# chenjianqu/dynamic_vins

Hardware: AMD Instinct MI355X
Metric: stereo frames/sec (track+BA) (higher is better)
Workload: dtype f64; 1 GPU; synthetic 1280x720 stereo @20 Hz + IMU @200 Hz, ZED intrinsics with distortion, figure-8 in a textured box room, max_cnt 250, min_dist 25, flow_back 1, 10 solver iterations, BA + marginalization on every frame; mode=raw, config=zed, parallelism=replicas x1 (independent sequences, no collective), landmarks_in_window=266, features_per_frame=250, warmup_requested=5, gpu_max_hw_queues=4, frames=resident in HBM before the timed region

## Files before the change

dynamic_vins_amd/csrc/be_api.hip:

```cpp
#include <algorithm>
#include "be_host.h"

static_assert(sizeof(dv_ba_factor) == sizeof(BeFactor), "public/private factor layouts must match");
static_assert(sizeof(dv_ba_lm) == sizeof(BeLm), "public/private landmark layouts must match");
static_assert(sizeof(dv_ba_prior) == sizeof(BePriorHdr), "public/private prior layouts must match");

int be_ensure(dv_ctx* ctx, int nfac) {
    BeWork& w = ctx->be;
    if (w.ready && nfac <= w.fac_cap) return 0;
    const int fac_cap = std::max(nfac, BE_MAX_LM * BE_MAX_OBS_FACTORS);
    size_t off = 0;
    auto take = [&](size_t bytes) { size_t o = off; off += (bytes + 255) / 256 * 256; return o; };
    const size_t n = BE_MAX_STATE;
    size_t o_ctl = take(sizeof(BeCtl)), o_x = take(sizeof(BeState)), o_imu = take(sizeof(BeImu) * BE_WIN), o_pr = take(sizeof(BePriorHdr)), o_i = take(4 * 4 * n),
           o_mt = take(4 * BE_MARG_TAB_INTS), o_lm = take(sizeof(BeLm) * BE_MAX_LM), o_fac = take(sizeof(BeFactor) * (size_t)fac_cap);
    const size_t upload_bytes = off;
    size_t o_c = take(sizeof(BeState)),
           o_pA = take(8 * (size_t)BE_MAX_PRIOR * BE_MAX_PRIOR), o_pb = take(8 * BE_MAX_PRIOR),
           o_pA2 = take(8 * (size_t)BE_MAX_PRIOR * BE_MAX_PRIOR), o_pb2 = take(8 * BE_MAX_PRIOR), o_ms = take(64), o_c0 = take(64),
           o_pk = take(8 * (size_t)BE_PK_SIZE * BE_PK_STRIDE), o_io = take(8 * (size_t)BE_WIN * IMU_OUT_STRIDE), o_po = take(8 * (BE_MAX_PRIOR + 1)),
           o_cc = take(8 * (BE_MAX_LM + BE_WIN + 1)), o_ob = take(4 * BE_MAX_LM), o_hd = take(8 * n * n), o_sc = take(8 * n * n), o_g = take(8 * 2 * n),
           o_pk1 = take(8 * (size_t)BE_PK_SIZE * BE_PK_STRIDE), o_io1 = take(8 * (size_t)BE_WIN * IMU_OUT_STRIDE), o_po1 = take(8 * (BE_MAX_PRIOR + 1)),
           o_hd1 = take(8 * n * n), o_sc1 = take(8 * n * n), o_g1 = take(8 * 2 * n),
           o_v = take(8 * 4 * n), o_vl = take(8 * 4 * (size_t)BE_MAX_LM);
// ... 267 lines not shown
    BeEvalArgs ea{};
    ea.ctl = w.ctl; ea.x = w.x; ea.cand = w.cand; ea.fac = w.fac; ea.lm = w.lm; ea.imu = w.imu; ea.prior = w.prior; ea.priorA = w.priorA; ea.priorb = w.priorb;
    ea.dims = d; ea.g_norm = P->g_norm; ea.cand_cost = w.cand_cost; ea.lm_obs = w.lm_obs; ea.prior_c0 = w.prior_c0 + w.prior_cur;
    ea.lm_lo = 0; ea.lm_hi = P->nlm;
    if (P->free_blocks & 3) {
        if (ctx->dist.transport != 0) DV_FAIL("dv_ba_solve: free extrinsic / td blocks are not built for the landmark-sharded window");
        if (xt.on) {
            DV_CHECK(w.xpk_buf.ensure(2 * 8 * (size_t)BX_SIZE * BE_PK_STRIDE));
            xt.xpk[0] = (double*)w.xpk_buf.p; xt.xpk[1] = xt.xpk[0] + (size_t)BX_SIZE * BE_PK_STRIDE;
        }
    }
    BeShard sh{};
    if (ctx->dist.transport != 0) {
        const DvDist& dd = ctx->dist;
        sh.on = 1; sh.rank = dd.rank; sh.world = dd.world;
        sh.cap = std::max(1, (P->nlm + dd.world - 1) / dd.world);
        sh.lo = std::min(P->nlm, dd.rank * sh.cap); sh.hi = std::min(P->nlm, sh.lo + sh.cap);
        sh.len = BE_XS_LEN;
        sh.xsend = (double*)dd.xsend.p; sh.xrecv = (const double*)dd.xrecv.p;
        sh.qf[0] = (double*)dd.qf.p; sh.qf[1] = sh.qf[0] + BE_QF_LEN;
        ea.lm_lo = sh.lo; ea.lm_hi = sh.hi;
    }
    for (int k = 0; k < 2; ++k) { ea.packets[k] = w.packets[k]; ea.imu_out[k] = w.imu_out[k]; ea.prior_out[k] = w.prior_out[k]; }
    BeSolveArgs sa{};
    sa.ctl = w.ctl; sa.x = w.x; sa.cand = w.cand; sa.lm = w.lm; sa.imu = w.imu; sa.prior = w.prior; sa.priorA = w.priorA; sa.dims = d;
    sa.cand_cost = w.cand_cost; sa.lm_obs = w.lm_obs;
    for (int k = 0; k < 2; ++k) { sa.packets[k] = w.packets[k]; sa.imu_out[k] = w.imu_out[k]; sa.prior_out[k] = w.prior_out[k]; sa.Hd[k] = w.Hd[k]; sa.Sc[k] = w.Sc[k]; sa.gvec[k] = w.gvec[k]; }
    sa.scale_p = w.scale_p; sa.diag_p = w.diag_p; sa.grad_p = w.grad_p; sa.gn_p = w.gn_p; sa.scale_l = w.scale_l; sa.diag_l = w.diag_l; sa.grad_l = w.grad_l; sa.gn_l = w.gn_l;
    sa.prior_col = w.prior_col; sa.col_kind = w.col_kind; sa.col_frame = w.col_frame; sa.col_comp = w.col_comp;
    sa.xnorm2_extra = P->x_norm2_extra; sa.sh = sh; sa.xt = xt;
    sa.ldl_mf16 = 0;
    if (!w.ldl_generic && !(P->free_blocks & 3)) {
        uint8_t plan[64];
        if (be_mf16_plan(d.nstate, plan)) { std::memcpy(sa.ldl_col0, plan, sizeof(plan)); sa.ldl_mf16 = 1; }
    }
    pd.rej_on = false;
    if (fused && fused->want_reject && w.gpu_reject && P->nlm > 0) {
        if (!w.rej_pinned) DV_CHECK(hipHostMalloc((void**)&w.rej_pinned, BE_MAX_LM, hipHostMallocDefault));
        BeRejectArgs& r = pd.rej;
        r.st = w.cand; r.fac = w.fac; r.lm = w.lm; r.nlm = P->nlm; r.nframes = P->nframes; r.focal = fused->rej_focal; r.flags = w.rej_pinned;
        std::memcpy(r.ric, fused->rej_ric, sizeof(r.ric)); std::memcpy(r.tic, fused->rej_tic, sizeof(r.tic));
        r.ex_from_state = (P->free_blocks & 1) ? 1 : 0; r.pad = 0;
        pd.rej_on = true;
    }
    pd.xt = xt; pd.copy_ex_td = (P->free_blocks & 3) != 0;
    pd.ea = ea; pd.sa = sa; pd.fused_present = fused != nullptr; pd.fuse_accept_gauge = fused != nullptr && !ctx->batch && !sh.on ; pd.max_iters = P->max_iters; pd.g_norm = P->g_norm; pd.nframes = P->nframes; pd.use_imu = P->use_imu; pd.nlm = P->nlm;
    pd.want_raw_pose = fused && fused->want_raw_pose;
    if (fused) { std::memcpy(pd.gauge_R0, fused->R0, sizeof(pd.gauge_R0)); std::memcpy(pd.gauge_ypr0, fused->ypr0, sizeof(pd.gauge_ypr0)); std::memcpy(pd.gauge_P0, fused->P0, sizeof(pd.gauge_P0)); }
    pd.do_marg = do_marg; pd.state_bytes = state_bytes; pd.nxt = 1 - w.prior_cur;
    if (eval_only) {
        be_launch_eval(ea, BE_EVAL_X, s); be_launch_eval_ext(ea, xt, BE_EVAL_X, s);
        be_launch_reduce(sa, 0, s); be_launch_reduce_ext(sa, 0, s);
        if (sh.on) { if (be_exchange(ctx, (size_t)sh.len, s)) return -1; be_launch_shard_finalize(sa, 0, s); }
        DV_CHECK(hipGetLastError());
        return 0;
    }
    if (w.debug_hash_log && fused) {
        if (!w.dbg_pinned) DV_CHECK(hipHostMalloc((void**)&w.dbg_pinned, 64, hipHostMallocDefault));
        const size_t up_bytes = w.up_fac + sizeof(BeFactor) * (size_t)P->nfac;
        be_dbg_hash(w.block.p, up_bytes & ~(size_t)7, w.dbg_pinned + 0, s);
        const bool pv = P->prior && P->prior->valid;
        if (pv) { be_dbg_hash(w.priorA, 8 * (size_t)P->prior->n * P->prior->n, w.dbg_pinned + 1, s); be_dbg_hash(w.priorb, 8 * (size_t)P->prior->n, w.dbg_pinned + 2, s); } else { w.dbg_pinned[1] = 0; w.dbg_pinned[2] = 0; }
    }
    const int first_slots = w.debug_short_first_pass ? std::max(1, P->max_iters - 2) : P->max_iters;
    if (ctx->batch && fused && !sh.on) {
        pd.deferred = true; pd.first_slots = first_slots;
        pd.active = true; pd.t_begin = t_begin; pd.t_up = t_up; pd.t_enq = t_up;
// ... 190 lines not shown
```

dynamic_vins_amd/csrc/be_debug.hip:

```cpp
#include <algorithm>
#include "be_host.h"

__global__ __launch_bounds__(256) void be_dbg_hash_kernel(const unsigned long long* __restrict__ p, size_t words, unsigned long long* __restrict__ out) {
    __shared__ unsigned long long sh[256];
    unsigned long long h = 1469598103934665603ull;
    for (size_t i = threadIdx.x; i < words; i += 256) { h ^= p[i]; h *= 1099511628211ull; }
    sh[threadIdx.x] = h;
    __syncthreads();
    if (threadIdx.x == 0) { unsigned long long t = 1469598103934665603ull; for (int k = 0; k < 256; ++k) { t ^= sh[k]; t *= 1099511628211ull; } *out = t; }
}
struct BeDbgJob { const unsigned long long* p[BeWork::DBG_RANGES]; unsigned long long words[BeWork::DBG_RANGES]; unsigned long long* out; };
__global__ __launch_bounds__(256) void be_dbg_hash_multi_kernel(BeDbgJob j) {
    __shared__ unsigned long long sh[256];
    const unsigned long long* p = j.p[blockIdx.x]; const unsigned long long words = j.words[blockIdx.x];
    unsigned long long h = 1469598103934665603ull;
    for (unsigned long long i = threadIdx.x; i < words; i += 256) { h ^= p[i]; h *= 1099511628211ull; }
    sh[threadIdx.x] = h;
    __syncthreads();
    if (threadIdx.x == 0) { unsigned long long t = 1469598103934665603ull; for (int k = 0; k < 256; ++k) { t ^= sh[k]; t *= 1099511628211ull; } j.out[blockIdx.x] = t; }
}
void be_dbg_stage(dv_ctx* c, int it, int kind, hipStream_t s) {
    BeWork& w = c->be;
    if (!w.debug_hash_log || it >= BeWork::DBG_SLOTS) return;
    const bool light = w.debug_hash_light;
// ... 16 lines not shown

extern "C" {

int dv_ba_debug_dev_log(dv_ctx* ctx, unsigned long long* rows7, int cap, int* n_rows) {
    if (!ctx) return -1;
    const int n = (int)(ctx->be.dbg_dev_log.size() / 7);
    if (n_rows) *n_rows = n;
    if (rows7) std::memcpy(rows7, ctx->be.dbg_dev_log.data(), sizeof(unsigned long long) * 7 * (size_t)std::min(n, std::max(cap, 0)));
    return 0;
}

int dv_ba_debug_slot_log(dv_ctx* ctx, unsigned long long* vals, long long cap_vals, long long* n_vals, int* row_len) {
    if (!ctx) return -1;
    const long long n = (long long)ctx->be.dbg_slot_log.size();
    if (n_vals) *n_vals = n;
    if (row_len) *row_len = BeWork::DBG_SLOTS * 5 * BeWork::DBG_RANGES;
    if (vals) std::memcpy(vals, ctx->be.dbg_slot_log.data(), sizeof(unsigned long long) * (size_t)std::min(n, std::max(cap_vals, 0ll)));
    return 0;
}

int dv_debug_set(dv_ctx* ctx, const char* key, int value) {
    if (!ctx || !key) return -1;
    if (std::strcmp(key, "short_first_pass") == 0) { ctx->be.debug_short_first_pass = value != 0; return 0; }
    if (std::strcmp(key, "peer_timeout_ms") == 0) { ctx->dist.peer_timeout_ticks = 100000ll * std::max(value, 1); return 0; }
    if (std::strcmp(key, "batch_single_eval") == 0) { ctx->be.debug_batch_single = (ctx->be.debug_batch_single & ~1) | (value ? 1 : 0); return 0; }
    if (std::strcmp(key, "batch_single_reduce") == 0) { ctx->be.debug_batch_single = (ctx->be.debug_batch_single & ~2) | (value ? 2 : 0); return 0; }
    if (std::strcmp(key, "batch_single_tail") == 0) { ctx->be.debug_batch_single = (ctx->be.debug_batch_single & ~8) | (value ? 8 : 0); return 0; }
    if (std::strcmp(key, "batch_single_solve") == 0) { ctx->be.debug_batch_single = (ctx->be.debug_batch_single & ~4) | (value ? 4 : 0); return 0; }
    if (std::strcmp(key, "hash_light") == 0) { ctx->be.debug_hash_light = value != 0; return 0; }
    if (std::strcmp(key, "hash_log") == 0) { ctx->be.debug_hash_log = value != 0; return 0; }
    if (std::strcmp(key, "wait_tail") == 0) { ctx->be.debug_wait_tail = value != 0; return 0; }
    if (std::strcmp(key, "gpu_reject") == 0) { ctx->be.gpu_reject = value != 0; return 0; }
    if (std::strcmp(key, "ldl_generic") == 0) { ctx->be.ldl_generic = value != 0; return 0; }
    DV_FAIL(std::string("dv_debug_set: unknown key ") + key);
}

}
```

dynamic_vins_amd/csrc/be_mf16.h:

```cpp
#pragma once
#include <hip/hip_runtime.h>
#include <cstdint>
#include "wave_dpp.h"

__device__ __forceinline__ void lds_barrier() { asm volatile("s_waitcnt lgkmcnt(0)\n\ts_barrier" ::: "memory"); }

__device__ __forceinline__ double fast_rcp(double d) {
    double r = __builtin_amdgcn_rcp(d);
    r = __builtin_fma(__builtin_fma(-d, r, 1.0), r, r);
    r = __builtin_fma(__builtin_fma(-d, r, 1.0), r, r);
    return r;
}

__device__ __forceinline__ void wave_lds_sync() { __builtin_amdgcn_fence(__ATOMIC_ACQ_REL, "wavefront"); __builtin_amdgcn_wave_barrier(); }

#define MF_SLOTS 5
#define MF_MAXNB 11
#define MF_RHO 1e300
typedef double mf_d4 __attribute__((ext_vector_type(4)));
__device__ __forceinline__ mf_d4 mf_mfma(double a, double b, mf_d4 c) { return __builtin_amdgcn_mfma_f64_16x16x4f64(a, b, c, 0, 0, 0); }
__device__ __forceinline__ int mf_tix(int I, int J, int NB) { return J * NB - (J * (J - 1)) / 2 + (I - J); }
template <int LANE> __device__ __forceinline__ double mf_rowbc(double v) { return dpp_f64<0x150 + LANE, 0xf>(v); }
__device__ __forceinline__ double mf_sel4(int rho, double v0, double v1, double v2, double v3) {
    const bool b0 = (rho & 1) != 0, b1 = (rho & 2) != 0;
    const double t0 = b0 ? v1 : v0, t1 = b0 ? v3 : v2;
    return b1 ? t1 : t0;
}
__device__ __forceinline__ int mf_wave() { return __builtin_amdgcn_readfirstlane(threadIdx.x >> 6); }
struct MfLds { double* Tl; double* gat; double* dv; double* iv; double* yv; };

template <int Q, bool RR>
__device__ __forceinline__ void mf_diag_substep(mf_d4& T, mf_d4& Wt, double* gat, double* dv16, double* iv16, int c0, double* yk) {
    constexpr int P = 4 * Q;
    const int lane = threadIdx.x & 63, c = lane & 15, rho = lane >> 4;
    gat[lane] = T[Q];
    wave_lds_sync();
    const double g0 = gat[c], g1 = gat[16 + c], g2 = gat[32 + c], g3 = gat[48 + c];
    const double d0 = gat[P], a10 = gat[16 + P], a11 = gat[16 + P + 1], a20 = gat[32 + P], a21 = gat[32 + P + 1], a22 = gat[32 + P + 2];
    const double a30 = gat[48 + P], a31 = gat[48 + P + 1], a32 = gat[48 + P + 2], a33 = gat[48 + P + 3];
    wave_lds_sync();
    const double i0 = RR ? (d0 > 1e-8 ? fast_rcp(d0) : 0.0) : fast_rcp(d0);
    const double l10 = a10 * i0, l20 = a20 * i0, l30 = a30 * i0;
    const double d1 = __builtin_fma(-l10, a10, a11), i1 = RR ? (d1 > 1e-8 ? fast_rcp(d1) : 0.0) : fast_rcp(d1);
    const double t21 = __builtin_fma(-l20, a10, a21), t31 = __builtin_fma(-l30, a10, a31);
    const double l21 = t21 * i1, l31 = t31 * i1;
    const double d2 = __builtin_fma(-l21, t21, __builtin_fma(-l20, a20, a22)), i2 = RR ? (d2 > 1e-8 ? fast_rcp(d2) : 0.0) : fast_rcp(d2);
    const double t32 = __builtin_fma(-l31, t21, __builtin_fma(-l30, a20, a32));
    const double l32 = t32 * i2;
    const double d3 = __builtin_fma(-l32, t32, __builtin_fma(-l31, t31, __builtin_fma(-l30, a30, a33))), i3 = RR ? (d3 > 1e-8 ? fast_rcp(d3) : 0.0) : fast_rcp(d3);
    const double p0 = g0, p1 = __builtin_fma(-p0, l10, g1);
    const double p2 = __builtin_fma(-p1, l21, __builtin_fma(-p0, l20, g2));
    const double p3 = __builtin_fma(-p2, l32, __builtin_fma(-p1, l31, __builtin_fma(-p0, l30, g3)));
    const double lh0 = c > P ? p0 * i0 : 0.0, lh1 = c > P + 1 ? p1 * i1 : 0.0, lh2 = c > P + 2 ? p2 * i2 : 0.0, lh3 = c > P + 3 ? p3 * i3 : 0.0;
    T = mf_mfma(-mf_sel4(rho, lh0, lh1, lh2, lh3), mf_sel4(rho, p0, p1, p2, p3), T);
    const double w20 = __builtin_fma(l21, l10, -l20), w31 = __builtin_fma(l32, l21, -l31);
    const double w30 = __builtin_fma(-l32, w20, __builtin_fma(l31, l10, -l30));
    const double z0 = -__builtin_fma(lh3, w30, __builtin_fma(lh2, w20, __builtin_fma(-lh1, l10, lh0)));
    const double z1 = -__builtin_fma(lh3, w31, __builtin_fma(-lh2, l21, lh1));
    const double z2 = -__builtin_fma(-lh3, l32, lh2);
    const double wq = Wt[Q];
    Wt = mf_mfma(mf_sel4(rho, z0, z1, z2, -lh3), wq, Wt);
    if (lane == 0) {
        mf_d4 dd = { d0, d1, d2, d3 }, ii = { i0, i1, i2, i3 };
        *reinterpret_cast<mf_d4*>(dv16 + P) = dd; *reinterpret_cast<mf_d4*>(iv16 + P) = ii;
    }
    if (lane == c0) { mf_d4 yy = { lh0, lh1, lh2, lh3 }; *reinterpret_cast<mf_d4*>(yk + P) = yy; }
}
template <bool RR = false>
__device__ __forceinline__ void mf_diag_factor(mf_d4& T, const MfLds& m, int k, int NB, int n, int* s_fail) {
    const int lane = threadIdx.x & 63, c = lane & 15, rho = lane >> 4, wave = mf_wave();
    __builtin_amdgcn_s_setprio(3);
    mf_d4 Wt;
#pragma unroll
    for (int r = 0; r < 4; ++r) Wt[r] = (rho + 4 * r == c) ? 1.0 : 0.0;
    double* gat = m.gat + wave * 64;
    const int nv = n - 16 * k, c0 = (nv >= 0 && nv < 16) ? nv : -1;
    mf_diag_substep<0, RR>(T, Wt, gat, m.dv + 16 * k, m.iv + 16 * k, c0, m.yv + 16 * k);
    if (c0 < 0 || c0 >= 4) mf_diag_substep<1, RR>(T, Wt, gat, m.dv + 16 * k, m.iv + 16 * k, c0, m.yv + 16 * k);
    if (c0 < 0 || c0 >= 8) mf_diag_substep<2, RR>(T, Wt, gat, m.dv + 16 * k, m.iv + 16 * k, c0, m.yv + 16 * k);
    if (c0 < 0 || c0 >= 12) mf_diag_substep<3, RR>(T, Wt, gat, m.dv + 16 * k, m.iv + 16 * k, c0, m.yv + 16 * k);
    *reinterpret_cast<mf_d4*>(m.Tl + (size_t)mf_tix(k, k, NB) * 256 + lane * 4) = Wt;
    {
        double* wt = m.gat + 768;
#pragma unroll
        for (int r = 0; r < 4; ++r) wt[((((c & 3) << 4) + rho + 4 * r) << 2) + (c >> 2)] = Wt[r];
    }
    __builtin_amdgcn_s_setprio(0);
}
__device__ __forceinline__ void mf_diag(mf_d4& T, const MfLds& m, int k, int NB, int n, int* s_fail) { mf_diag_factor<false>(T, m, k, NB, n, s_fail); }
__device__ __forceinline__ void mf_slots(const uint8_t* plan, int wave, int NB, int (&sI)[5], int (&sJ)[5]) {
    sI[0] = sJ[0] = wave < NB ? wave : -1;
    const uint32_t w4 = reinterpret_cast<const uint32_t*>(plan)[wave];
#pragma unroll
    for (int s = 1; s < 5; ++s) { const int b = (int)((w4 >> (8 * (s - 1))) & 0xFFu); sI[s] = b == 0xFF ? -1 : (b >> 4); sJ[s] = b == 0xFF ? -1 : (b & 15); }
}

template <bool RR, class After>
__device__ __forceinline__ void mf16_factor_core(mf_d4 (&U)[MF_SLOTS], const uint8_t* plan, int n, const MfLds& m, int* s_fail, After after_update) {
    const int lane = threadIdx.x & 63, wave = mf_wave(), c = lane & 15, rho = lane >> 4;
    const int NB = (n + 16) >> 4, IB = n >> 4, c0 = n & 15;
    int sI[MF_SLOTS], sJ[MF_SLOTS];
    mf_slots(plan, wave, NB, sI, sJ);
    if (wave == 0) mf_diag_factor<RR>(U[0], m, 0, NB, n, s_fail);
    lds_barrier();
    auto panel = [&](mf_d4& T, int I, int k) -> mf_d4 {
        const mf_d4 wf = *reinterpret_cast<const mf_d4*>(m.gat + 768 + lane * 4);
        double ivr[4];
#pragma unroll
        for (int q = 0; q < 4; ++q) ivr[q] = m.iv[16 * k + rho + 4 * q];
        mf_d4 Y = { 0.0, 0.0, 0.0, 0.0 };
#pragma unroll
        for (int q = 0; q < 4; ++q) Y = mf_mfma(wf[q], T[q], Y);
        const mf_d4 Y0 = Y;
#pragma unroll
// ... 39 lines not shown
```

dynamic_vins_amd/csrc/be_solve.hip:

```cpp
#include <hip/hip_runtime.h>
#include <cfloat>
#include <algorithm>
#include <cstring>
#include <cstdlib>
#include "be_kernels.h"
#include "dev_once.h"
#include "wave_dpp.h"
#include "be_mf16.h"

using namespace be;

#ifdef BE_RED_TS
__device__ long long be_red_ts[64];
#define RTS(k) do { if (threadIdx.x == 0) be_red_ts[k] = wall_clock64(); } while (0)
extern "C" int dv_debug_red_ts(long long* out) { return hipMemcpyFromSymbol(out, HIP_SYMBOL(be_red_ts), sizeof(long long) * 64) == hipSuccess ? 0 : -1; }
#else
#define RTS(k) do {} while (0)
#endif
#define RED_THREADS 448
#define RED_PAIRS (BE_NF * (BE_NF + 1) / 2)
__device__ const unsigned char RED_PAIR_TAB[RED_PAIRS] = {
    150, 152, 51, 132, 98, 166, 170, 112, 147, 85, 68, 65, 32, 168, 49, 167, 118, 153, 66, 129, 96, 130, 165, 144, 33, 148, 67, 48, 102, 162, 161, 0, 97,
    133, 50, 16, 101, 134, 17, 119, 99, 84, 114, 64, 80, 100, 163, 160, 145, 149, 115, 131, 82, 164, 81, 151, 113, 117, 116, 128, 34, 136, 83, 169, 146, 135 };
__device__ __forceinline__ void red_pair(int bx, int& fi, int& fj) { const int t = RED_PAIR_TAB[bx]; fi = t >> 4; fj = t & 15; }
// ... 650 lines not shown
    const int NBR = (n + 3) >> 2, bi = i >> 2, bj = j >> 2;
    const bool in = i < n;
    return Sc[in ? (size_t)(bj * NBR - bj * (bj - 1) / 2 + bi - bj) * 16 + (i & 3) * 4 + (j & 3) : 0];
}
__device__ __forceinline__ double mf_finish(double raw, const double* v_s, const double* v_d, const double* rhs, int n, double mu, int i, int j) {
    const int hi = i > j ? i : j, lo = i > j ? j : i, hc = hi < n ? hi : n - 1, lc = lo < n ? lo : n - 1;
    const double s_hi = v_s[hc], s_lo = v_s[lc], d_hi = v_d[hc];
    const double body = s_hi * s_lo * raw + (i == j ? mu * d_hi * d_hi : 0.0);
    const double row_n = lo == n ? MF_RHO : s_lo * rhs[lc];
    return hi < n ? body : (hi == n ? row_n : (hi == lo ? 1.0 : 0.0));
}
__device__ __forceinline__ void mf_prefetch(const double* __restrict__ Sc, const uint8_t* plan, int n, mf_d4 (&U)[5]) {
    const int lane = threadIdx.x & 63, wave = mf_wave(), c = lane & 15, rho = lane >> 4;
    int sI[5], sJ[5];
    mf_slots(plan, wave, (n + 16) >> 4, sI, sJ);
    const int NBR = (n + 3) >> 2;
#pragma unroll
    for (int s = 0; s < 5; ++s) {
        if (sI[s] > sJ[s]) {
            const int i = min(16 * sI[s] + c, n - 1);
            const int lane_off = ((i >> 2) << 4) + ((i & 3) << 2) + rho;
#pragma unroll
            for (int r = 0; r < 4; ++r) {
                const int bj = 4 * sJ[s] + r;
                const int bjc = bj < NBR ? bj : 0;
                U[s][r] = Sc[(size_t)((bjc * NBR - bjc * (bjc - 1) / 2 - bjc) << 4) + lane_off];
            }
        } else {
#pragma unroll
            for (int r = 0; r < 4; ++r) U[s][r] = sI[s] >= 0 ? mf_raw(Sc, n, 16 * sI[s] + c, 16 * sJ[s] + rho + 4 * r) : 0.0;
        }
    }
}
template <class Side, class Side0>
__device__ __forceinline__ bool ldlt_mf16(mf_d4 (&U)[MF_SLOTS], const uint8_t* plan, int n, double mu, const double* v_s, const double* v_d, const double* rhs, const MfLds& m, int* s_fail, Side side, Side0 side0) {
    const int tid = threadIdx.x, lane = tid & 63, wave = mf_wave(), c = lane & 15, rho = lane >> 4;
    const int NB = (n + 16) >> 4, IB = n >> 4, c0 = n & 15;
    int sI[MF_SLOTS], sJ[MF_SLOTS];
    mf_slots(plan, wave, NB, sI, sJ);
    TS(21);
#pragma unroll
    for (int s = 0; s < MF_SLOTS; ++s) {
        if (sI[s] > sJ[s]) {
            const int i = 16 * sI[s] + c;
            const double si = v_s[min(i, n - 1)];
#pragma unroll
            for (int r = 0; r < 4; ++r) {
                const int j = 16 * sJ[s] + rho + 4 * r;
                const double sj = v_s[j];
                const double body = si * sj * U[s][r];
                U[s][r] = i < n ? body : (i == n ? sj * rhs[j] : 0.0);
            }
        } else {
#pragma unroll
            for (int r = 0; r < 4; ++r) U[s][r] = sI[s] >= 0 ? mf_finish(U[s][r], v_s, v_d, rhs, n, mu, 16 * sI[s] + c, 16 * sJ[s] + rho + 4 * r) : 0.0;
        }
    }
    TS(22);
    for (int i = tid; i < 16 * NB; i += SOL_THREADS) m.yv[i] = 0.0;
    if (tid == 0) *s_fail = 0;
#ifdef BE_SOLVE_TS
    if (tid == 0) { be_dbg_ts[19] = 0; be_dbg_ts[20] = 0; be_dbg_ts[32] = 0; be_dbg_ts[33] = 0; be_dbg_ts[34] = 0; be_dbg_ts[35] = 0; }
#endif
    lds_barrier();
    TS(4);
    const int k_side = -1;
    if (wave == 0) { mf_diag(U[0], m, 0, NB, n, s_fail); if (k_side < 0) side0(); }
    else if (k_side < 0) side(0);
    lds_barrier();
#ifdef BE_SOLVE_TS
    long long t_prev = wall_clock64(), acc_panel = 0, acc_update = 0;
    if (tid == 0) be_dbg_ts[16] = t_prev - be_dbg_ts[4];
#endif
    auto panel = [&](mf_d4& T, int I, int k) -> mf_d4 {
        const mf_d4 wf = *reinterpret_cast<const mf_d4*>(m.gat + 768 + lane * 4);
        double ivr[4];
#pragma unroll
        for (int q = 0; q < 4; ++q) ivr[q] = m.iv[16 * k + rho + 4 * q];
        mf_d4 Y = { 0.0, 0.0, 0.0, 0.0 };
#pragma unroll
        for (int q = 0; q < 4; ++q) Y = mf_mfma(wf[q], T[q], Y);
        const mf_d4 Y0 = Y;
#pragma unroll
        for (int r = 0; r < 4; ++r) Y[r] *= ivr[r];
        T = Y;
        *reinterpret_cast<mf_d4*>(m.Tl + (size_t)mf_tix(I, k, NB) * 256 + lane * 4) = Y;
        if (I == IB && c == c0) {
#pragma unroll
            for (int r = 0; r < 4; ++r) m.yv[16 * k + rho + 4 * r] = Y[r];
        }
        return Y0;
    };
    for (int k = 0; k + 1 < NB; ++k) {
        if (wave == k + 1) {
            __builtin_amdgcn_s_setprio(3);
#ifdef BE_SOLVE_TS
            const long long t_c0 = wall_clock64();
#endif
            const mf_d4 Y0 = panel(U[1], k + 1, k);
#ifdef BE_SOLVE_TS
            __builtin_amdgcn_s_waitcnt(0xc07f); const long long t_c1 = wall_clock64();
#endif
#pragma unroll
            for (int q = 0; q < 4; ++q) U[0] = mf_mfma(U[1][q], -Y0[q], U[0]);
#ifdef BE_SOLVE_TS
            asm volatile("s_nop 15\n\ts_nop 3\n\tv_mov_b64 %0, %0" : "+v"(U[0][0])); const long long t_c2 = wall_clock64();
#endif
            if (k + 2 < NB) lds_barrier();
#ifdef BE_SOLVE_TS
            const long long t_u = wall_clock64();
            if (lane == 0) { be_dbg_ts[32] += t_c0 - t_prev; be_dbg_ts[33] += t_c1 - t_c0; be_dbg_ts[34] += t_c2 - t_c1; be_dbg_ts[35] += t_u - t_c2; }
#endif
            mf_diag(U[0], m, k + 1, NB, n, s_fail);
#ifdef BE_SOLVE_TS
            if (lane == 0) { be_dbg_ts[19] += wall_clock64() - t_u; be_dbg_ts[20] += t_u - t_prev; }
#endif
            lds_barrier();
        } else {
#pragma unroll
            for (int s = 1; s < MF_SLOTS; ++s) if (sJ[s] == k) panel(U[s], sI[s], k);
            if (k + 2 < NB) lds_barrier();
#ifdef BE_SOLVE_TS
            { const long long t = wall_clock64(); acc_panel += t - t_prev; t_prev = t; }
#endif
            double dk[4];
// ... 126 lines not shown
        const double xk = lane_bcast(xs, kt - u - 64 * SEG);
        x0 = __builtin_fma(-(SEG == 0 ? m[u] : cr[u][0]), xk, x0);
        if (SEG >= 1) x1 = __builtin_fma(-(SEG == 1 ? m[u] : cr[u][1]), xk, x1);
        if (SEG >= 2) x2 = __builtin_fma(-m[u], xk, x2);
    }
}
template <int SEG, int R>
__device__ __forceinline__ int bs_segment(const double* Lm, int k, int lane, double& x0, double& x1, double& x2) {
    const int kend = 64 * SEG + R - 1;
    double ca[R][3], cb[R][3];
    bs_ld<SEG, R>(Lm, k, lane, ca);
    for (; k >= kend; k -= 2 * R) {
        if (k - R >= kend) bs_ld<SEG, R>(Lm, k - R, lane, cb);
        __builtin_amdgcn_sched_barrier(0);
        bs_ap<SEG, R>(ca, k, lane, x0, x1, x2);
        __builtin_amdgcn_sched_barrier(0);
        if (k - R >= kend) {
            if (k - 2 * R >= kend) bs_ld<SEG, R>(Lm, k - 2 * R, lane, ca);
            __builtin_amdgcn_sched_barrier(0);
            bs_ap<SEG, R>(cb, k - R, lane, x0, x1, x2);
            __builtin_amdgcn_sched_barrier(0);
        }
    }
    return 64 * SEG - 1;
}
template <int ROWS>
__device__ __forceinline__ void bs_rows(const double* Lm, int kt, int lane, double& x0, double& x1, double& x2) {
    const int seg = kt >> 6;
    if (seg == 0) bs_chunk<0, ROWS>(Lm, kt, lane, x0, x1, x2);
    else if (seg == 1) bs_chunk<1, ROWS>(Lm, kt, lane, x0, x1, x2);
    else bs_chunk<2, ROWS>(Lm, kt, lane, x0, x1, x2);
}

template <int NSLOT, bool MF16>
__global__ __launch_bounds__(SOL_THREADS) void be_solve_kernel(BeSolveArgs a, int spec) {
    constexpr bool SHARD = false;
#include "be_solve_body.inc"
}
template <int NSLOT, bool MF16>
__global__ __launch_bounds__(SOL_THREADS) void be_solve_batch_kernel(const BeSolveArgs* __restrict__ tab, int spec) {
    const BeSolveArgs& a = tab[blockIdx.x];
    constexpr bool SHARD = false;
#include "be_solve_body.inc"
}
__global__ __launch_bounds__(SOL_THREADS) void be_solve_shard_kernel(BeSolveArgs a, int spec) {
    constexpr int NSLOT = 1; constexpr bool MF16 = true, SHARD = true;
#include "be_solve_body.inc"
}

static size_t solve_smem(int n) {
    const size_t tri = (size_t)n * (n + 1) / 2;
    return (tri + 9 * (size_t)n + 72 + 80 + 8 + 1536) * sizeof(double);
}
static size_t solve_smem_mf16(int n) {
    const size_t NB = ((size_t)n + 16) >> 4, nt = NB * (NB + 1) / 2;
    return (std::max<size_t>(nt * 256, 3072) + 9 * (size_t)n + 72 + 80 + 8 + 1024 + 3 * 16 * NB) * sizeof(double);
}
bool be_mf16_plan(int n, uint8_t* plan , bool check_solve_lds) {
    const int NB = (n + 16) >> 4, W = SOL_THREADS / 64;
    if (NB > MF_MAXNB || (check_solve_lds && solve_smem_mf16(n) > 160 * 1024 - 512)) return false;
    int load[SOL_THREADS / 64] = { 0 };
    std::memset(plan, 0xFF, (size_t)W * 4);
    for (int j = 1; j < NB; ++j) plan[j * 4 + load[j]++] = (uint8_t)((j << 4) | (j - 1));
    for (int J = 0; J < NB - 1; ++J) {
        int el[SOL_THREADS / 64], ne = 0;
        for (int w = 0; w < W; ++w) if ((w == 0 || w >= NB || J < w) && w != J + 1 && load[w] < 4) el[ne++] = w;
        auto key = [&](int w) { return ((1 <= w && w < NB) ? w - 1 : NB) * 1024 + load[w] * 32 + w; };
        std::sort(el, el + ne, [&](int x, int y) { return key(x) < key(y); });
        if (ne < NB - 2 - J) return false;
        for (int t = 0, I = J + 2; I < NB; ++I, ++t) { const int w = el[t]; plan[w * 4 + load[w]++] = (uint8_t)((I << 4) | J); }
    }
    return true;
}

int be_launch_solve(const BeSolveArgs& a, int spec, hipStream_t s) {
    static DevOnce once;
    if (once.run([] {
            if (hipFuncSetAttribute(reinterpret_cast<const void*>(be_solve_kernel<1, false>), hipFuncAttributeMaxDynamicSharedMemorySize, (int)solve_smem(BE_MAX_STATE)) != hipSuccess) return 1;
            if (hipFuncSetAttribute(reinterpret_cast<const void*>(be_solve_kernel<2, false>), hipFuncAttributeMaxDynamicSharedMemorySize, (int)solve_smem(BE_MAX_STATE)) != hipSuccess) return 1;
            return hipFuncSetAttribute(reinterpret_cast<const void*>(be_solve_kernel<1, true>), hipFuncAttributeMaxDynamicSharedMemorySize, 160 * 1024 - 512) != hipSuccess ? 1 : 0; })) return -1;
    const int nbr = (a.dims.nstate + 3) / 4;
    if (a.sh.on) {
        if (!a.ldl_mf16 || solve_smem_mf16(a.dims.nstate) > 160 * 1024 - 1024) return -2;
        static DevOnce once_s;
        if (once_s.run([] { return hipFuncSetAttribute(reinterpret_cast<const void*>(be_solve_shard_kernel), hipFuncAttributeMaxDynamicSharedMemorySize, 160 * 1024 - 1024) != hipSuccess ? 1 : 0; })) return -1;
        hipLaunchKernelGGL(be_solve_shard_kernel, dim3(1), dim3(SOL_THREADS), solve_smem_mf16(a.dims.nstate), s, a, spec);
        return 0;
    }
    if (a.ldl_mf16) hipLaunchKernelGGL((be_solve_kernel<1, true>), dim3(1), dim3(SOL_THREADS), solve_smem_mf16(a.dims.nstate), s, a, spec);
    else if (nbr * (nbr + 1) / 2 <= SOL_THREADS) hipLaunchKernelGGL((be_solve_kernel<1, false>), dim3(1), dim3(SOL_THREADS), solve_smem(a.dims.nstate), s, a, spec);
    else hipLaunchKernelGGL((be_solve_kernel<2, false>), dim3(1), dim3(SOL_THREADS), solve_smem(a.dims.nstate), s, a, spec);
    return 0;
}

int be_launch_solve_batch(const BeSolveArgs* tab_dev, int n_win, int max_n, int spec, hipStream_t s) {
    static DevOnce once;
    if (once.run([] { return hipFuncSetAttribute(reinterpret_cast<const void*>(be_solve_batch_kernel<1, true>), hipFuncAttributeMaxDynamicSharedMemorySize, 160 * 1024 - 512) != hipSuccess ? 1 : 0; })) return -1;
    hipLaunchKernelGGL((be_solve_batch_kernel<1, true>), dim3(n_win), dim3(SOL_THREADS), solve_smem_mf16(max_n), s, tab_dev, spec);
    return 0;
}

__global__ __launch_bounds__(256) void be_accept_kernel(BeSolveArgs a) { be_accept_body(a); }
void be_launch_accept(const BeSolveArgs& a, hipStream_t s) { hipLaunchKernelGGL(be_accept_kernel, dim3(1), dim3(256), 0, s, a); }

int be_solve_prepare() {
    hipFuncAttributes fa;
    if (hipFuncGetAttributes(&fa, reinterpret_cast<const void*>(be_reduce_kernel)) != hipSuccess) return -1;
    static DevOnce once;
    return once.run([] { return hipFuncSetAttribute(reinterpret_cast<const void*>(be_solve_kernel<1, true>), hipFuncAttributeMaxDynamicSharedMemorySize, 160 * 1024 - 512) != hipSuccess ? 1 : 0; }) ? -1 : 0;
}
```

dynamic_vins_amd/csrc/be_solve_body.inc:

```
    extern __shared__ __attribute__((aligned(16))) double sm[];
    BeCtl* ctl = a.ctl;
    BeCtl c = *ctl;
    const int n = a.dims.nstate, nlm = a.dims.nlm, tid = threadIdx.x;
    const int lm0 = SHARD ? a.sh.lo : 0, nown = SHARD ? a.sh.hi - a.sh.lo : nlm;
    if (c.done) return;
    __shared__ int s_pcol[BE_NF], s_scol[BE_NF];
    if (tid < BE_NF) { s_pcol[tid] = tid < a.dims.nframes ? a.dims.pose_col[tid] : -1; s_scol[tid] = tid < a.dims.nframes ? a.dims.sb_col[tid] : -1; }
    __shared__ int s_xcol[MF16 ? 1 : 16]; __shared__ double qx[MF16 ? 1 : 16];
    bool xt_on = false;
    if constexpr (!MF16) { xt_on = a.xt.on != 0; if (tid >= 64 && tid < 80) s_xcol[tid - 64] = (xt_on && tid - 64 < BE_NX) ? a.xt.xcol[tid - 64] : -1; }
    TS(15);
    const int cur_spec = (spec && c.pending) ? (c.cur ^ 1) : c.cur;
    double dec_cv[4] = { 0.0, 0.0, 0.0, 0.0 };
    if (MF16 && spec && c.pending && tid < 256) {
        const int ncost0 = nlm + a.dims.nimu + 1;
#pragma unroll
        for (int u = 0; u < 4; ++u) dec_cv[u] = a.cand_cost[tid + 256 * u < ncost0 ? tid + 256 * u : 0];
    }
    mf_d4 mfU[MF_SLOTS];
    double pre_h = 0.0, pre_g0 = 0.0, pre_g1 = 0.0, pre_s = 0.0;
    if (MF16 && !(c.reuse && !(spec && c.pending))) {
        mf_prefetch(a.Sc[cur_spec], reinterpret_cast<const uint8_t*>(a.ldl_col0), n, mfU);
        if (tid < n) { pre_h = a.Hd[cur_spec][(size_t)tid * n + tid]; pre_g0 = a.gvec[cur_spec][tid]; pre_g1 = a.gvec[cur_spec][n + tid]; pre_s = a.scale_p[tid]; }
    }
// ... 167 lines not shown
                if (tid == 0) part += prior_out[0];
                if (SHARD && tid == 0) part += qfc[BE_QF_A + 10];
                const double xc = block_sum(part, red);
                if (tid == 0) { ctl->x_cost = xc; ctl->initial_cost = xc; }
            }
            {
                double gm = 0;
                for (int i = tid; i < n; i += SOL_THREADS) gm = fmax(gm, fabs(gvec[i]));
                if (!SHARD) for (int l = tid; l < nlm; l += SOL_THREADS) gm = fmax(gm, fabs(BE_PK(pk, BE_PK_G, l)));
                else if (tid == 0) gm = fmax(gm, qfc[BE_QF_A + 11]);
    #pragma unroll
                for (int o = 32; o > 0; o >>= 1) gm = fmax(gm, __shfl_xor(gm, o));
                __syncthreads();
                if ((tid & 63) == 0) red[tid >> 6] = gm;
                __syncthreads();
                gm = 0; for (int k = 0; k < SOL_THREADS / 64; ++k) gm = fmax(gm, red[k]);
                __syncthreads();
                if (gm <= 1e-10) { if (tid == 0) { ctl->done = 1; ctl->termination = 1; ctl->first = 0; } return true; }
            }
            TS(1);
            if (lm_live) {
                const int l = lmi;
                const double h = BE_PK(pk, BE_PK_H, l), gl = BE_PK(pk, BE_PK_G, l), s = a.scale_l[l];
                double d2 = h * s * s; d2 = fmin(fmax(d2, 1e-6), 1e32);
                const double d = sqrt(d2);
                a.diag_l[l] = d; a.grad_l[l] = gl * s / d;
                lm_h = h; lm_g = gl; lm_scale = s; lm_diag = d; lm_grad = gl * s / d;
            }
            return false;
        };
        if (!MF16) { if (cost_and_tolerance()) return; }
        TS(3);
        bool ok_f;
        if (MF16) ok_f = ldlt_mf16(mfU, reinterpret_cast<const uint8_t*>(a.ldl_col0), n, mu, v_s, v_d, v_x, mf, &s_fail, [&](int excl) { side_sums(tid < 64 * excl ? tid : tid - 64, SOL_THREADS - 64, false); },
                                   [&]() { lm_diag_own(); if ((tid & 63) == 0) { red[tid >> 6] = 0.0; red[16 + (tid >> 6)] = 0.0; } });
        else ok_f = ldlt_blocked<NSLOT>(a.Sc[c.cur], gvec, n, mu, v_s, v_d, Lm, PL, PD, dinfo, zfin, dvec, &s_fail);
        if (!ok_f) {
            if (MF16) { if (cost_and_tolerance()) return; }
            if (tid == 0) {
                ctl->mu = mu * 10.0; ctl->chol_fail = 1; ctl->first = 0; ctl->alpha_valid = 0;
                ctl->slots = c.slots + 1; ctl->reuse = 0; ctl->need_eval = 0; ctl->pending = 0;
                if (mu * 10.0 > 1.0) { ctl->done = 1; ctl->termination = 2; }
            }
            return;
        }
        TS(6);
        if (MF16) bs_mf16(reinterpret_cast<const uint8_t*>(a.ldl_col0), n, mf, v_x);
        else if ((tid >> 6) == 0) {
            __builtin_amdgcn_s_setprio(3);
            const int lane = tid & 63, nn = n;
            double x0 = lane < nn ? zfin[lane] / dvec[lane] : 0.0;
            double x1 = 64 + lane < nn ? zfin[64 + lane] / dvec[64 + lane] : 0.0;
            double x2 = 128 + lane < nn ? zfin[128 + lane] / dvec[128 + lane] : 0.0;
            int k = nn - 1;
            for (; k >= 0 && ((k + 1) & 7); --k) bs_rows<1>(Lm, k, lane, x0, x1, x2);
            if (k >= 128 + BS_R - 1) k = bs_segment<2, BS_R>(Lm, k, lane, x0, x1, x2);
            if (k >= 64 + BS_R - 1) k = bs_segment<1, BS_R>(Lm, k, lane, x0, x1, x2);
            if (k >= BS_R - 1) k = bs_segment<0, BS_R>(Lm, k, lane, x0, x1, x2);
            __builtin_amdgcn_s_setprio(0);
            if (lane < nn) v_x[lane] = x0;
            if (64 + lane < nn) v_x[64 + lane] = x1;
            if (128 + lane < nn) v_x[128 + lane] = x2;
        }
        lds_barrier();
        if (MF16) {
            double gm = 0, xc = 0;
            for (int k = 0; k < SOL_THREADS / 64; ++k) { gm = fmax(gm, red[k]); xc += red[16 + k]; }
// ... 234 lines not shown
```

dynamic_vins_amd/csrc/dv_ctx.h:

```cpp
#pragma once
#include "dv_internal.h"
#include "be_types.h"
#include "be_kernels.h"
#include <cmath>
#include <cstring>
#include <chrono>
#include <deque>
#include <map>
#include <memory>
#include <mutex>
#include <string>
#include <vector>

struct DevBuf {
    void* p = nullptr; size_t bytes = 0;
    hipError_t ensure(size_t n) {
        if (n <= bytes) return hipSuccess;
        if (p) (void)hipFree(p);
        p = nullptr; bytes = 0;
        hipError_t e = hipMalloc(&p, n);
        if (e == hipSuccess) bytes = n;
        return e;
    }
    void release() { if (p) (void)hipFree(p); p = nullptr; bytes = 0; }
// ... 53 lines not shown
    hipEvent_t ev_state_ext = nullptr;
    bool fuse_accept_gauge = false;
    bool active = false, trivial = false, do_marg = false, fused_present = false, marg_in_flight = false, marg_check_due = false; int scal_slot = 0, check_slot = 0; size_t state_bytes = 0; int nxt = 0; MargPlan pl;
    BeExt xt{}; bool copy_ex_td = false;
    BeEvalArgs ea; BeSolveArgs sa; int max_iters = 0, nframes = 0, use_imu = 0, nlm = 0; double g_norm = 0, gauge_R0[9], gauge_ypr0[3], gauge_P0[3];
    std::chrono::steady_clock::time_point t_begin, t_up, t_enq;
};

struct BeWork {
    std::unique_ptr<BePending> pend = std::make_unique<BePending>();
    bool ready = false;
    DevBuf block;
    BeCtl* ctl = nullptr; BeState* x = nullptr; BeState* cand = nullptr;
    BeFactor* fac = nullptr; BeLm* lm = nullptr; BeImu* imu = nullptr; BePriorHdr* prior = nullptr; double* priorA = nullptr; double* priorb = nullptr;
    double* packets[2] = { nullptr, nullptr }; double* imu_out[2] = { nullptr, nullptr }; double* prior_out[2] = { nullptr, nullptr }; double* cand_cost = nullptr; int32_t* lm_obs = nullptr;
    double* Hd[2] = { nullptr, nullptr }; double* Sc[2] = { nullptr, nullptr }; double* gvec[2] = { nullptr, nullptr };
    double* scale_p = nullptr; double* diag_p = nullptr; double* grad_p = nullptr; double* gn_p = nullptr;
    double* scale_l = nullptr; double* diag_l = nullptr; double* grad_l = nullptr; double* gn_l = nullptr;
    int32_t* prior_col = nullptr; int32_t* col_kind = nullptr; int32_t* col_frame = nullptr; int32_t* col_comp = nullptr;
    int fac_cap = 0;
    DevBuf marg_buf;
    DevBuf xpk_buf;
    void* pinned = nullptr; size_t pinned_bytes = 0;
    size_t up_ctl = 0, up_x = 0, up_imu = 0, up_prior = 0, up_idx = 0, up_mt = 0, up_lm = 0, up_fac = 0, dl_off = 0;
    double* priorA_buf[2] = { nullptr, nullptr }; double* priorb_buf[2] = { nullptr, nullptr }; int prior_cur = 0;
    bool prior_resident = false;
    hipEvent_t ev_state = nullptr;
    double* prior_c0 = nullptr;
    int marg_form = 0;
    DevBuf eig_spec; bool eig_ran = false;
    int32_t* marg_tab = nullptr; double* marg_scal = nullptr;
    long long marg_checked = 0; double marg_last[4] = { 0, 0, 0, 0 };
    long long marg_clamped = 0;
    bool debug_short_first_pass = false, ldl_generic = false, debug_wait_tail = false; int debug_batch_single = 0; bool debug_hash_log = false, debug_hash_light = false;
    std::vector<unsigned long long> dbg_dev_log; unsigned long long* dbg_pinned = nullptr; unsigned long long dbg_solve_no = 0;
    static constexpr int DBG_RANGES = 16, DBG_SLOTS = 16;
    unsigned long long* dbg_slots = nullptr; std::vector<unsigned long long> dbg_slot_log;
    bool gpu_reject = true; uint8_t* rej_pinned = nullptr;
    std::vector<const double*> sqrt_hint;
};

bool be_imu_sqrt_info(const double* cov15x15, double* U15x15);

struct BeFused {
    int marg_mode = -1;
    double R0[9], ypr0[3], P0[3];
    dv_ba_prior new_prior;
    double diag[4] = { 0, 0, 0, 0 };
    bool want_raw_pose = false;
    bool want_reject = false; double rej_ric[2][9], rej_tic[2][3], rej_focal = 0; const uint8_t* rej_flags = nullptr;
    double raw_pose[77];
};
int be_solve_fused(dv_ctx* ctx, dv_ba_problem* P, dv_ba_summary* summary, BeFused* fused);
void be_batch_detach(dv_ctx* ctx);
struct DvFrontBatch;
DvFrontBatch*& be_batch_front(struct dv_batch* B);
const std::vector<dv_ctx*>& be_batch_members(struct dv_batch* B);
void dv_front_batch_release(DvFrontBatch* F);
void dv_front_batch_sync(DvFrontBatch* F);
void* be_staging_factors(dv_ctx* ctx, int* cap);
int be_solve_fused_begin(dv_ctx* ctx, dv_ba_problem* P, BeFused* fused);
int be_solve_fused_end(dv_ctx* ctx, dv_ba_problem* P, dv_ba_summary* summary, BeFused* fused);
struct dv_obj_problem;
struct ObjPending {
    bool active = false; void* pinned = nullptr; size_t pinned_bytes = 0, up_bytes = 0; hipEvent_t ev = nullptr; hipStream_t stream = nullptr; int V = 0, nblk = 0, n_obj = 0;
    void release() { if (pinned) (void)hipHostFree(pinned); pinned = nullptr; pinned_bytes = 0; if (ev) (void)hipEventDestroy(ev); ev = nullptr; active = false; }
};
// ... 103 lines not shown
```

Baseline: 1197 frames/s.

## Replace block barriers in MFMA LDLT with LDS dataflow flags between waves

The blocked MFMA LDL^T factorization in the BA solve kernel now coordinates its waves through per-column LDS counters and flags, replacing workgroup-wide barriers at every column step. The diagonal wave waits only for the panel count it needs, and the other waves wait only for the diagonal flag or panel completion before doing their trailing updates. This targets barrier stalls on the serial critical path of the small dense solve that runs every iteration. It adds spin-wait loops and depends on the ordering of relaxed atomics, and the old barrier path is kept behind a debug flag.

```diff
diff --git a/dynamic_vins_amd/csrc/be_api.hip b/dynamic_vins_amd/csrc/be_api.hip
--- a/dynamic_vins_amd/csrc/be_api.hip
+++ b/dynamic_vins_amd/csrc/be_api.hip
@@ -323,7 +323,7 @@
     sa.ldl_mf16 = 0;
     if (!w.ldl_generic && !(P->free_blocks & 3)) {
         uint8_t plan[64];
-        if (be_mf16_plan(d.nstate, plan)) { std::memcpy(sa.ldl_col0, plan, sizeof(plan)); sa.ldl_mf16 = 1; }
+        if (be_mf16_plan(d.nstate, plan)) { std::memcpy(sa.ldl_col0, plan, sizeof(plan)); sa.ldl_mf16 = w.ldl_barriers ? 2 : 1; }
     }
     pd.rej_on = false;
     if (fused && fused->want_reject && w.gpu_reject && P->nlm > 0) {
diff --git a/dynamic_vins_amd/csrc/be_debug.hip b/dynamic_vins_amd/csrc/be_debug.hip
--- a/dynamic_vins_amd/csrc/be_debug.hip
+++ b/dynamic_vins_amd/csrc/be_debug.hip
@@ -72,6 +72,7 @@
     if (std::strcmp(key, "wait_tail") == 0) { ctx->be.debug_wait_tail = value != 0; return 0; }
     if (std::strcmp(key, "gpu_reject") == 0) { ctx->be.gpu_reject = value != 0; return 0; }
     if (std::strcmp(key, "ldl_generic") == 0) { ctx->be.ldl_generic = value != 0; return 0; }
+    if (std::strcmp(key, "ldl_barriers") == 0) { ctx->be.ldl_barriers = value != 0; return 0; }
     DV_FAIL(std::string("dv_debug_set: unknown key ") + key);
 }
 
diff --git a/dynamic_vins_amd/csrc/be_mf16.h b/dynamic_vins_amd/csrc/be_mf16.h
--- a/dynamic_vins_amd/csrc/be_mf16.h
+++ b/dynamic_vins_amd/csrc/be_mf16.h
@@ -13,6 +13,23 @@
 }
 
 __device__ __forceinline__ void wave_lds_sync() { __builtin_amdgcn_fence(__ATOMIC_ACQ_REL, "wavefront"); __builtin_amdgcn_wave_barrier(); }
+
+#define MF_FLAGS 16
+__device__ __forceinline__ int mf_flag_peek(const int* f) { return __hip_atomic_load(f, __ATOMIC_RELAXED, __HIP_MEMORY_SCOPE_WORKGROUP); }
+__device__ __forceinline__ void mf_flag_set(int* f, int v, int lane) {
+    asm volatile("s_waitcnt lgkmcnt(0)" ::: "memory");
+    if (lane == 0) __hip_atomic_store(f, v, __ATOMIC_RELAXED, __HIP_MEMORY_SCOPE_WORKGROUP);
+}
+__device__ __forceinline__ void mf_flag_add(int* f, int v, int lane) {
+    asm volatile("s_waitcnt lgkmcnt(0)" ::: "memory");
+    if (lane == 0) __hip_atomic_fetch_add(f, v, __ATOMIC_RELAXED, __HIP_MEMORY_SCOPE_WORKGROUP);
+}
+template <bool CHAIN>
+__device__ __forceinline__ void mf_flag_wait(const int* f, int v, int seen = -1) {
+    int cur = __builtin_amdgcn_readfirstlane(seen);
+    while (cur < v) { cur = __builtin_amdgcn_readfirstlane(mf_flag_peek(f)); if (!CHAIN && cur < v) __builtin_amdgcn_s_sleep(1); }
+    asm volatile("" ::: "memory");
+}
 
 #define MF_SLOTS 5
 #define MF_MAXNB 11
@@ -66,8 +83,8 @@
     }
     if (lane == c0) { mf_d4 yy = { lh0, lh1, lh2, lh3 }; *reinterpret_cast<mf_d4*>(yk + P) = yy; }
 }
-template <bool RR = false>
-__device__ __forceinline__ void mf_diag_factor(mf_d4& T, const MfLds& m, int k, int NB, int n, int* s_fail) {
+template <bool RR = false, bool DF = false>
+__device__ __forceinline__ void mf_diag_factor(mf_d4& T, const MfLds& m, int k, int NB, int n, int* s_fail, const int* img_cnt = nullptr, int img_need = 0) {
     const int lane = threadIdx.x & 63, c = lane & 15, rho = lane >> 4, wave = mf_wave();
     __builtin_amdgcn_s_setprio(3);
     mf_d4 Wt;
@@ -76,10 +93,13 @@
     double* gat = m.gat + wave * 64;
     const int nv = n - 16 * k, c0 = (nv >= 0 && nv < 16) ? nv : -1;
     mf_diag_substep<0, RR>(T, Wt, gat, m.dv + 16 * k, m.iv + 16 * k, c0, m.yv + 16 * k);
+    int img_seen = 0;
+    if (DF && img_need > 0) img_seen = mf_flag_peek(img_cnt);
     if (c0 < 0 || c0 >= 4) mf_diag_substep<1, RR>(T, Wt, gat, m.dv + 16 * k, m.iv + 16 * k, c0, m.yv + 16 * k);
     if (c0 < 0 || c0 >= 8) mf_diag_substep<2, RR>(T, Wt, gat, m.dv + 16 * k, m.iv + 16 * k, c0, m.yv + 16 * k);
     if (c0 < 0 || c0 >= 12) mf_diag_substep<3, RR>(T, Wt, gat, m.dv + 16 * k, m.iv + 16 * k, c0, m.yv + 16 * k);
     *reinterpret_cast<mf_d4*>(m.Tl + (size_t)mf_tix(k, k, NB) * 256 + lane * 4) = Wt;
+    if (DF && img_need > 0) mf_flag_wait<true>(img_cnt, img_need, img_seen);
     {
         double* wt = m.gat + 768;
 #pragma unroll
diff --git a/dynamic_vins_amd/csrc/be_solve.hip b/dynamic_vins_amd/csrc/be_solve.hip
--- a/dynamic_vins_amd/csrc/be_solve.hip
+++ b/dynamic_vins_amd/csrc/be_solve.hip
@@ -706,7 +706,7 @@
         }
     }
 }
-template <class Side, class Side0>
+template <bool DF, class Side, class Side0>
 __device__ __forceinline__ bool ldlt_mf16(mf_d4 (&U)[MF_SLOTS], const uint8_t* plan, int n, double mu, const double* v_s, const double* v_d, const double* rhs, const MfLds& m, int* s_fail, Side side, Side0 side0) {
     const int tid = threadIdx.x, lane = tid & 63, wave = mf_wave(), c = lane & 15, rho = lane >> 4;
     const int NB = (n + 16) >> 4, IB = n >> 4, c0 = n & 15;
@@ -733,15 +733,22 @@
     TS(22);
     for (int i = tid; i < 16 * NB; i += SOL_THREADS) m.yv[i] = 0.0;
     if (tid == 0) *s_fail = 0;
+    __shared__ int s_mf_flag[DF ? MF_FLAGS : 1];
+    if (DF && tid < MF_FLAGS) s_mf_flag[tid] = 0;
 #ifdef BE_SOLVE_TS
     if (tid == 0) { be_dbg_ts[19] = 0; be_dbg_ts[20] = 0; be_dbg_ts[32] = 0; be_dbg_ts[33] = 0; be_dbg_ts[34] = 0; be_dbg_ts[35] = 0; }
 #endif
     lds_barrier();
     TS(4);
     const int k_side = -1;
-    if (wave == 0) { mf_diag(U[0], m, 0, NB, n, s_fail); if (k_side < 0) side0(); }
+    int* const dflag = s_mf_flag; int* const pcnt = s_mf_flag + (DF ? 1 : 0);
+    if (wave == 0) {
+        mf_diag_factor<false, DF>(U[0], m, 0, NB, n, s_fail);
+        if (DF) mf_flag_set(dflag, 1, lane);
+        if (k_side < 0) side0();
+    }
     else if (k_side < 0) side(0);
-    lds_barrier();
+    if (!DF) lds_barrier();
 #ifdef BE_SOLVE_TS
     long long t_prev = wall_clock64(), acc_panel = 0, acc_update = 0;
     if (tid == 0) be_dbg_ts[16] = t_prev - be_dbg_ts[4];
@@ -765,6 +772,64 @@
         }
         return Y0;
     };
+    if constexpr (DF) {
+    for (int k = 0; k + 1 < NB; ++k) {
+        const int np_col = NB - 1 - k;
+        if (wave == k + 1) {
+#ifdef BE_SOLVE_TS
+            const long long t_w = wall_clock64();
+#endif
+            mf_flag_wait<true>(dflag, k + 1);
+            __builtin_amdgcn_s_setprio(3);
+#ifdef BE_SOLVE_TS
+            const long long t_c0 = wall_clock64();
+#endif
+            const mf_d4 Y0 = panel(U[1], k + 1, k);
+#ifdef BE_SOLVE_TS
+            __builtin_amdgcn_s_waitcnt(0xc07f); const long long t_c1 = wall_clock64();
+#endif
+#pragma unroll
+            for (int q = 0; q < 4; ++q) U[0] = mf_mfma(U[1][q], -Y0[q], U[0]);
+#ifdef BE_SOLVE_TS
+            asm volatile("s_nop 15\n\ts_nop 3\n\tv_mov_b64 %0, %0" : "+v"(U[0][0])); const long long t_c2 = wall_clock64();
+#endif
+            mf_flag_add(pcnt + k, 1, lane);
+#ifdef BE_SOLVE_TS
+            const long long t_u = wall_clock64();
+            if (lane == 0) { be_dbg_ts[32] += t_c0 - t_w; be_dbg_ts[33] += t_c1 - t_c0; be_dbg_ts[34] += t_c2 - t_c1; be_dbg_ts[35] += t_u - t_c2; }
+#endif
+            mf_diag_factor<false, true>(U[0], m, k + 1, NB, n, s_fail, pcnt + k, np_col);
+            mf_flag_set(dflag, k + 2, lane);
+#ifdef BE_SOLVE_TS
+            if (lane == 0) { be_dbg_ts[19] += wall_clock64() - t_u; be_dbg_ts[20] += t_u - t_c0; }
+#endif
+        } else {
+            int np = 0; bool upd = false;
+#pragma unroll
+            for (int s = 0; s < MF_SLOTS; ++s) { np += (s >= 1 && sJ[s] == k) ? 1 : 0; upd = upd || sJ[s] > k; }
+            if (np) {
+                mf_flag_wait<false>(dflag, k + 1);
+#pragma unroll
+                for (int s = 1; s < MF_SLOTS; ++s) if (sJ[s] == k) panel(U[s], sI[s], k);
+                mf_flag_add(pcnt + k, np, lane);
+            }
+            if (upd) {
+                mf_flag_wait<false>(pcnt + k, np_col);
+                double dk[4];
+#pragma unroll
+                for (int q = 0; q < 4; ++q) dk[q] = -m.dv[16 * k + rho + 4 * q];
+#pragma unroll
+                for (int s = 0; s < MF_SLOTS; ++s) if (sJ[s] > k) {
+                    const mf_d4 a = *reinterpret_cast<const mf_d4*>(m.Tl + (size_t)mf_tix(sJ[s], k, NB) * 256 + lane * 4);
+                    const mf_d4 b = *reinterpret_cast<const mf_d4*>(m.Tl + (size_t)mf_tix(sI[s], k, NB) * 256 + lane * 4);
+#pragma unroll
+                    for (int q = 0; q < 4; ++q) U[s] = mf_mfma(a[q], dk[q] * b[q], U[s]);
+                }
+            }
+        }
+    }
+    lds_barrier();
+    } else
     for (int k = 0; k + 1 < NB; ++k) {
         if (wave == k + 1) {
             __builtin_amdgcn_s_setprio(3);
@@ -957,19 +1022,19 @@
     else bs_chunk<2, ROWS>(Lm, kt, lane, x0, x1, x2);
 }
 
-template <int NSLOT, bool MF16>
+template <int NSLOT, bool MF16, bool BARRIERS = false>
 __global__ __launch_bounds__(SOL_THREADS) void be_solve_kernel(BeSolveArgs a, int spec) {
-    constexpr bool SHARD = false;
+    constexpr bool SHARD = false, MF_DF = MF16 && !BARRIERS;
 #include "be_solve_body.inc"
 }
 template <int NSLOT, bool MF16>
 __global__ __launch_bounds__(SOL_THREADS) void be_solve_batch_kernel(const BeSolveArgs* __restrict__ tab, int spec) {
     const BeSolveArgs& a = tab[blockIdx.x];
-    constexpr bool SHARD = false;
+    constexpr bool SHARD = false, MF_DF = MF16;
 #include "be_solve_body.inc"
 }
 __global__ __launch_bounds__(SOL_THREADS) void be_solve_shard_kernel(BeSolveArgs a, int spec) {
-    constexpr int NSLOT = 1; constexpr bool MF16 = true, SHARD = true;
+    constexpr int NSLOT = 1; constexpr bool MF16 = true, SHARD = true, MF_DF = false;
 #include "be_solve_body.inc"
 }
 
@@ -1003,6 +1068,7 @@
     if (once.run([] {
             if (hipFuncSetAttribute(reinterpret_cast<const void*>(be_solve_kernel<1, false>), hipFuncAttributeMaxDynamicSharedMemorySize, (int)solve_smem(BE_MAX_STATE)) != hipSuccess) return 1;
             if (hipFuncSetAttribute(reinterpret_cast<const void*>(be_solve_kernel<2, false>), hipFuncAttributeMaxDynamicSharedMemorySize, (int)solve_smem(BE_MAX_STATE)) != hipSuccess) return 1;
+            if (hipFuncSetAttribute(reinterpret_cast<const void*>(be_solve_kernel<1, true, true>), hipFuncAttributeMaxDynamicSharedMemorySize, 160 * 1024 - 512) != hipSuccess) return 1;
             return hipFuncSetAttribute(reinterpret_cast<const void*>(be_solve_kernel<1, true>), hipFuncAttributeMaxDynamicSharedMemorySize, 160 * 1024 - 512) != hipSuccess ? 1 : 0; })) return -1;
     const int nbr = (a.dims.nstate + 3) / 4;
     if (a.sh.on) {
@@ -1012,7 +1078,8 @@
         hipLaunchKernelGGL(be_solve_shard_kernel, dim3(1), dim3(SOL_THREADS), solve_smem_mf16(a.dims.nstate), s, a, spec);
         return 0;
     }
-    if (a.ldl_mf16) hipLaunchKernelGGL((be_solve_kernel<1, true>), dim3(1), dim3(SOL_THREADS), solve_smem_mf16(a.dims.nstate), s, a, spec);
+    if (a.ldl_mf16 == 2) hipLaunchKernelGGL((be_solve_kernel<1, true, true>), dim3(1), dim3(SOL_THREADS), solve_smem_mf16(a.dims.nstate), s, a, spec);
+    else if (a.ldl_mf16) hipLaunchKernelGGL((be_solve_kernel<1, true>), dim3(1), dim3(SOL_THREADS), solve_smem_mf16(a.dims.nstate), s, a, spec);
     else if (nbr * (nbr + 1) / 2 <= SOL_THREADS) hipLaunchKernelGGL((be_solve_kernel<1, false>), dim3(1), dim3(SOL_THREADS), solve_smem(a.dims.nstate), s, a, spec);
     else hipLaunchKernelGGL((be_solve_kernel<2, false>), dim3(1), dim3(SOL_THREADS), solve_smem(a.dims.nstate), s, a, spec);
     return 0;
diff --git a/dynamic_vins_amd/csrc/be_solve_body.inc b/dynamic_vins_amd/csrc/be_solve_body.inc
--- a/dynamic_vins_amd/csrc/be_solve_body.inc
+++ b/dynamic_vins_amd/csrc/be_solve_body.inc
@@ -223,7 +223,7 @@
         if (!MF16) { if (cost_and_tolerance()) return; }
         TS(3);
         bool ok_f;
-        if (MF16) ok_f = ldlt_mf16(mfU, reinterpret_cast<const uint8_t*>(a.ldl_col0), n, mu, v_s, v_d, v_x, mf, &s_fail, [&](int excl) { side_sums(tid < 64 * excl ? tid : tid - 64, SOL_THREADS - 64, false); },
+        if (MF16) ok_f = ldlt_mf16<MF_DF>(mfU, reinterpret_cast<const uint8_t*>(a.ldl_col0), n, mu, v_s, v_d, v_x, mf, &s_fail, [&](int excl) { side_sums(tid < 64 * excl ? tid : tid - 64, SOL_THREADS - 64, false); },
                                    [&]() { lm_diag_own(); if ((tid & 63) == 0) { red[tid >> 6] = 0.0; red[16 + (tid >> 6)] = 0.0; } });
         else ok_f = ldlt_blocked<NSLOT>(a.Sc[c.cur], gvec, n, mu, v_s, v_d, Lm, PL, PD, dinfo, zfin, dvec, &s_fail);
         if (!ok_f) {
diff --git a/dynamic_vins_amd/csrc/dv_ctx.h b/dynamic_vins_amd/csrc/dv_ctx.h
--- a/dynamic_vins_amd/csrc/dv_ctx.h
+++ b/dynamic_vins_amd/csrc/dv_ctx.h
@@ -109,7 +109,7 @@
     int32_t* marg_tab = nullptr; double* marg_scal = nullptr;
     long long marg_checked = 0; double marg_last[4] = { 0, 0, 0, 0 };
     long long marg_clamped = 0;
-    bool debug_short_first_pass = false, ldl_generic = false, debug_wait_tail = false; int debug_batch_single = 0; bool debug_hash_log = false, debug_hash_light = false;
+    bool debug_short_first_pass = false, ldl_generic = false, ldl_barriers = false, debug_wait_tail = false; int debug_batch_single = 0; bool debug_hash_log = false, debug_hash_light = false;
     std::vector<unsigned long long> dbg_dev_log; unsigned long long* dbg_pinned = nullptr; unsigned long long dbg_solve_no = 0;
     static constexpr int DBG_RANGES = 16, DBG_SLOTS = 16;
     unsigned long long* dbg_slots = nullptr; std::vector<unsigned long long> dbg_slot_log;
```

After: 1225 frames/s, median of 6. +2.3%, better.
